# Kotomiya07/kuzushiji-vision

Measured on AMD Instinct MI355X. Metric: line-images/sec (train), higher is better.
Workload: dtype bf16; 1 GPU; TrOCR train step: ViT-B/16 (12L/768/12h/3072) on 64x640 crops (S_e=161) + RoBERTa decoder 6L/256/4h/768, V=4300 one-char vocab, labels [B,128], dropout 0.1, clip 1.0, RAdamScheduleFree; BASELINE.json configs[1]; per_gpu_batch=256, global_batch=256, parallelism=dp1

## Files before the change

include/kzv.h:

```cpp
#ifndef KZV_H
#define KZV_H
#include <stddef.h>
#include <stdint.h>

#ifdef __cplusplus
extern "C" {
#endif

#define KZV_OK 0
#define KZV_E_ARG (-1)
#define KZV_E_HIP (-2)
#define KZV_E_STATE (-3)

const char* kzv_last_error(void);
int kzv_version(void);

typedef struct kzv_config {
    int32_t image_h, image_w, patch_h, patch_w, channels;
    int32_t enc_hidden, enc_layers, enc_heads, enc_ffn;
    int32_t dec_hidden, dec_layers, dec_heads, dec_ffn;
    int32_t vocab, max_pos, type_vocab, pad_id;
    float enc_hidden_dropout, enc_attn_dropout, dec_hidden_dropout, dec_attn_dropout;
    float ln_eps;
} kzv_config;
// ... 342 lines not shown
                   float* dz, float* dgamma, float* dbeta, void* dy_bf16, int relu, int train, float* d_scratch, void* stream);
int kzv_ocr_maxpool_fwd(const void* x_bf16, void* out_bf16, unsigned char* idx, int N, int H, int W, int C, void* stream);
int kzv_ocr_maxpool_bwd(const float* dout, const unsigned char* idx, float* dx, int N, int H, int W, int C, void* stream);
int kzv_ocr_avgpool_fwd(const void* x_bf16, float* feat_f32, void* feat_bf16, int N, int HW, int C, void* stream);
int kzv_ocr_avgpool_bwd(const float* dfeat, float* dx, int N, int HW, int C, void* stream);
int kzv_ocr_lstm_cell_fwd(const float* gates, const float* b_hh, float* h_f32, void* h_bf16, int64_t ldh, int B, int H, void* stream);
int kzv_ocr_lstm_cell_bwd(const float* gates, const float* b_hh, const float* dh, int64_t lddh, void* dgates_bf16, int B, int H, void* stream);
int kzv_ocr_log_softmax(const float* x, float* lp, int rows, int C, void* stream);
int kzv_ocr_ctc(const float* lp, const int64_t* targets, int64_t ld_targets, const int64_t* input_lengths, const int64_t* target_lengths, int T,
                int B, int C, int blank, int zero_infinity, int max_target_len, float* d_scratch, float* d_nll, const float* d_gscale,
                float* d_dlogits, void* stream);
int kzv_ocr_smooth_l1_boxes(const float* pred, int max_boxes, const float* gt, int gt_boxes, const int32_t* counts, int B, float* d_loss,
                            float* d_dpred, void* stream);
int kzv_ocr_adam(float* p, const float* g, float* m, float* v, int64_t n, float lr, float beta1, float beta2, float eps, int step, void* stream);
int kzv_ocr_adam_dev(float* p, const float* g, float* m, float* v, int64_t n, float lr, float beta1, float beta2, float eps, const float* d_bc,
                     void* stream);
int kzv_ocr_cast_bf16(const float* x, void* out_bf16, int64_t n, void* stream);
int kzv_ocr_cast_transpose(const float* x, void* out_bf16, int rows, int cols, void* stream);

int kzv_prof_enable(int on, int capacity);
int kzv_prof_select(unsigned kind_mask);
int kzv_prof_collect(int kind, double* total_ms, double* total_flops, int64_t* launches);
int kzv_prof_sample(int stride);
int64_t kzv_prof_seen(int kind);
uint32_t kzv_drop_key(uint64_t seed, uint32_t site);

#define KZV_SITE_ENC_EMB 1u
#define KZV_SITE_ENC_LAYER(i, k) (16u + 4u * (uint32_t)(i) + (uint32_t)(k))
#define KZV_SITE_DEC_EMB 1000u
#define KZV_SITE_DEC_LAYER(i, k) (1016u + 8u * (uint32_t)(i) + (uint32_t)(k))

int kzv_debug_dropout_mask(uint32_t key, float p, int64_t rows, int64_t cols, int64_t ld_index, float* d_out, void* stream);
int kzv_debug_attn_dropout_mask(uint32_t key, float p, int64_t pairs, int32_t Sq, int32_t Sk, float* d_out, void* stream);

int kzv_set_cu_reserve(int n);
int kzv_get_cu_reserve(void);

int64_t kzv_scratch_growths(void);

typedef struct {
    int64_t src_off;
    int64_t tmp_off;
    int64_t hb_off, hk_off;
    int64_t vb_off, vk_off;
    int32_t in_h, in_w, new_h, new_w, paste_x, paste_y, hk_size, vk_size;
} kzv_line_desc;
int kzv_lanczos_coeffs(int in_size, int out_size, int32_t* bounds, int32_t* kk, int* ksize);
int kzv_preprocess_lines(const uint8_t* rgb, const kzv_line_desc* desc, const int32_t* coef, int n, int target_h, int target_w,
                         int64_t max_tmp_pixels, const float* lut256, uint8_t* tmp, float* out, void* stream);

typedef struct {
    float m[6];
    float blur[7];
    float contrast, brightness, noise_sigma;
    uint32_t noise_key;
    int32_t morph;
} kzv_augment_params;
int kzv_augment_lines(const float* in, const kzv_augment_params* params, int n, int H, int W, float* out, void* stream);

#ifdef __cplusplus
}
#endif
#endif
```

kuzushiji-vision_amd/csrc/gemm.hip:

```cpp
#include "kzv_common.h"
#include "../../include/kzv.h"
#include "kzv_host.h"
#include "gemm_nt.h"
#include "gemm_tn.h"

namespace {

constexpr int BK = 64;
constexpr int STAGE_BYTES = (128 + 128) * BK * 2;
constexpr int NT_LDS = 2 * STAGE_BYTES;

template <int N> __device__ __forceinline__ void wait_vmcnt() {
    if constexpr (N == 0) asm volatile("s_waitcnt vmcnt(0)" ::: "memory");
    else if constexpr (N == 4) asm volatile("s_waitcnt vmcnt(4)" ::: "memory");
    else if constexpr (N == 6) asm volatile("s_waitcnt vmcnt(6)" ::: "memory");
    else if constexpr (N == 8) asm volatile("s_waitcnt vmcnt(8)" ::: "memory");
    else if constexpr (N == 12) asm volatile("s_waitcnt vmcnt(12)" ::: "memory");
    else if constexpr (N == 16) asm volatile("s_waitcnt vmcnt(16)" ::: "memory");
    else static_assert(N == 0, "add the vmcnt literal");
}

template <int EPI, int WM, int WN, int NSTAGE, int KB, bool ASM_DMA>
__global__ __launch_bounds__(WM * WN * 64) void gemm_nt_kernel(const NtParams p) {
    constexpr int BM = WM * 64, BN = WN * 64, NW = WM * WN;
// ... 270 lines not shown
#pragma unroll
    for (int j = 0; j < 4; ++j)
#pragma unroll
        for (int i = 0; i < 4; ++i)
#pragma unroll
            for (int r = 0; r < 4; ++r) {
                const int n = wn * 64 + j * 16 + 4 * g + r, k = wk * 64 + i * 16 + l15;
                tile[n * 128 + ((((k >> 2) ^ (n & 31)) << 2) | (k & 3))] = acc[i][j][r];
            }
    __syncthreads();
    const bool interior = tnb * 128 + 128 <= p.n_store && tkb * 128 + 128 <= p.K;
    for (int it0 = 0; it0 < 64; it0 += 8) {
        float v[8];
#pragma unroll
        for (int u = 0; u < 8; ++u) {
            const int it = it0 + u;
            const int n = w * 32 + (it >> 1), k = (it & 1) * 64 + lane;
            v[u] = tile[n * 128 + ((((k >> 2) ^ (n & 31)) << 2) | (k & 3))];
        }
#pragma unroll
        for (int u = 0; u < 8; ++u) {
            const int it = it0 + u;
            const int n = w * 32 + (it >> 1), k = (it & 1) * 64 + lane;
            const int gn = tnb * 128 + n, gk = tkb * 128 + k;
            float* o = p.OUT + (int64_t)gn * p.ldo + gk;
            if (interior && p.splits > 1) atomicAdd(o, v[u]);
            else if (gn < p.n_store && gk < p.K) { if (p.splits == 1) *o += v[u]; else atomicAdd(o, v[u]); }
        }
    }
}

__global__ __launch_bounds__(256, 2) void gemm_tn_kernel(const TnParams p) { gemm_tn_body(p, blockIdx.x); }

constexpr int TN_GROUP_MAX = 40;
struct TnGroup { TnParams p[TN_GROUP_MAX]; int start[TN_GROUP_MAX + 1]; int n; };
__global__ __launch_bounds__(256, 2) void gemm_tn_group_kernel(const TnGroup g) {
    int i = 0;
#pragma unroll 1
    while (i + 1 < g.n && (int)blockIdx.x >= g.start[i + 1]) ++i;
    gemm_tn_body(g.p[i], (int)blockIdx.x - g.start[i]);
}

}

static int g_nt_schedule = -1;
static int g_nt_half_mask = -1;
static int nt_schedule() {
    if (g_nt_schedule < 0) {
        g_nt_schedule = kzv_env_int("KZV_NT_FREE", 0) != 0;
        if (kzv_env_int("KZV_NT_HALF", 0)) g_nt_schedule |= 2;
    }
    return g_nt_schedule;
}
static int nt_half_mask() {
    if (g_nt_half_mask < 0) g_nt_half_mask = kzv_env_int("KZV_NT_HALF_EPIS", 0x3f);
    return g_nt_half_mask;
}
extern "C" int kzv_set_nt_schedule(int n) { g_nt_schedule = n < 0 ? -1 : (n & 3); return KZV_OK; }
extern "C" int kzv_set_nt_half_epilogues(int mask) { g_nt_half_mask = mask; return KZV_OK; }

int kzv_nt_params(const kzv_gemm_nt_args* a, int epilogue, NtParams* out) {
    if (!a || !a->A || !a->B || !a->C) return kzv_fail(KZV_E_ARG, "gemm_nt: null operand");
    if (a->M <= 0 || a->N <= 0 || a->K <= 0) return kzv_fail(KZV_E_ARG, "gemm_nt: empty shape");
    if (a->K % 64) return kzv_fail(KZV_E_ARG, "gemm_nt: K must be a multiple of 64");
    if (a->N % 4 || a->ldc % 4) return kzv_fail(KZV_E_ARG, "gemm_nt: N and ldc must be multiples of 4");
    if (a->lda % 8 || a->ldb % 8) return kzv_fail(KZV_E_ARG, "gemm_nt: lda/ldb must be multiples of 8 (16-byte rows)");
    if (((uintptr_t)a->A | (uintptr_t)a->B | (uintptr_t)a->C) & 15) return kzv_fail(KZV_E_ARG, "gemm_nt: operands must be 16-byte aligned");
// ... 176 lines not shown
```

kuzushiji-vision_amd/csrc/gemm_tn.h:

```cpp
#pragma once
#include "kzv_common.h"

struct TnParams {
    const bf16_t* P; const bf16_t* Q; float* OUT; const void* zero16;
    int64_t ldp, ldq, ldo;
    int Mtok, N, K, n_store, splits, chunk;
    float* dbias;
};

inline bool tn_dma_offsets_fit(const TnParams& p) {
    return (uint64_t)64 * (uint64_t)p.ldp * 2 + (uint64_t)p.N * 2 <= 0xffffffffull && (uint64_t)64 * (uint64_t)p.ldq * 2 + (uint64_t)p.K * 2 <= 0xffffffffull;
}

int kzv_tn256_launch(const TnParams& p, hipStream_t s);

struct KzvTnFoldScope { explicit KzvTnFoldScope(hipStream_t stream); ~KzvTnFoldScope(); hipStream_t s; };

struct kzv_gemm_nt_args; struct kzv_gemm_tn_args;
int kzv_gemm_pair_launch(const kzv_gemm_nt_args* na, int epilogue, const kzv_gemm_tn_args* ta, hipStream_t s);
```

kuzushiji-vision_amd/csrc/gemm_tn256.hip:

```cpp
#include "kzv_common.h"
#include "../../include/kzv.h"
#include "kzv_host.h"
#include "gemm_tn.h"
#include "gemm_nt.h"
#include "gemm256_common.h"
#include "gemm_nt256p_body.h"
#include <vector>
#include <type_traits>

namespace {

constexpr int HT_BYTES = 64 * 256;
constexpr int BUF_BYTES = 4 * HT_BYTES;
constexpr int LDS_BYTES = 2 * BUF_BYTES;
constexpr int KP0 = 0, KP1 = 1, KQ0 = 2, KQ1 = 3;
#ifndef KZV_TN_F32_PARTIALS
constexpr size_t PART_FLOATS = 32768;
#else
constexpr size_t PART_FLOATS = 65536;
#endif

__global__ __launch_bounds__(512) void gemm_tn256_kernel(const TnParams p, float* part_ws) {
    extern __shared__ __attribute__((aligned(16))) char smem[];
    const int tid = threadIdx.x, lane = tid & 63;
    const int w = __builtin_amdgcn_readfirstlane(tid >> 6);
    const int g = lane >> 4, l15 = lane & 15;
    const int wr = w >> 2, wc = w & 3;
    const int tilesN = (p.N + 255) / 256, tilesK = (p.K + 255) / 256;
    const int per = tilesN * tilesK;
    const int id = xcd_remap(blockIdx.x, per * p.splits);
    const int split = id / per, rem = id - split * per;
    const int tnb = rem / tilesK, tkb = rem - tnb * tilesK;
    const int t_begin = split * p.chunk;
    const int t_end = min(p.Mtok, t_begin + p.chunk);
    const int nt = (t_end - t_begin) >> 6;

    const char* baseP = (const char*)(p.P + (int64_t)t_begin * p.ldp);
    const char* baseQ = (const char*)(p.Q + (int64_t)t_begin * p.ldq);
    const int64_t stepP = 64 * p.ldp * 2, stepQ = 64 * p.ldq * 2;
// ... 139 lines not shown
    }

    float* tile = (float*)smem;
    float* part = part_ws + (size_t)id * PART_FLOATS;
#pragma unroll
    for (int c = 0; c < 2; ++c) {
        __syncthreads();
#pragma unroll
        for (int j = 0; j < 4; ++j)
#pragma unroll
            for (int i = 0; i < 4; ++i)
#pragma unroll
                for (int r = 0; r < 4; ++r) {
                    const int ln = wr * 64 + j * 16 + 4 * g + r;
                    const int k = (i >> 1) * 128 + wc * 32 + (i & 1) * 16 + l15;
                    tile[ln * 256 + ((((k >> 2) ^ (ln & 31)) << 2) | (k & 3))] = acc[i][c * 4 + j][r];
                }
        __syncthreads();
#pragma unroll
        for (int it = 0; it < 16; ++it) {
            const int ln = w * 16 + it;
            const f32x4 v = *(const f32x4*)(tile + ln * 256 + ((lane ^ (ln & 31)) << 2));
            const int row = c * 128 + ln;
#ifndef KZV_TN_F32_PARTIALS
            typedef __attribute__((ext_vector_type(2))) unsigned u32x2p;
            __builtin_nontemporal_store((u32x2p){pack_bf2(v[0], v[1]), pack_bf2(v[2], v[3])}, (u32x2p*)((bf16_t*)part + row * 256 + lane * 4));
#else
            __builtin_nontemporal_store(v, (f32x4*)(part + row * 256 + lane * 4));
#endif
        }
    }
}

__device__ __forceinline__ void tn256f_body(const TnParams& p, float* const part, const int tnb, const int tkb, const int t_begin, const int nt,
                                            char* const smem) {
    const int tid = threadIdx.x, lane = tid & 63;
    const int w = __builtin_amdgcn_readfirstlane(tid >> 6);
    const int g = lane >> 4, l15 = lane & 15;
    const int wr = w >> 2, wc = w & 3;
    const int tilesK = (p.K + 255) / 256;

    const unsigned ldp2 = (unsigned)p.ldp * 2u, ldq2 = (unsigned)p.ldq * 2u;
    const char* baseP = (const char*)(p.P + (int64_t)t_begin * p.ldp);
    const char* baseQ = (const char*)(p.Q + (int64_t)t_begin * p.ldq);
    const int64_t stepP = 64 * (int64_t)ldp2, stepQ = 64 * (int64_t)ldq2;
    unsigned cP[2], cQ[2];
    {
        const int r = w * 4 + (lane >> 4);
        const int col2 = ((lane & 15) ^ ((r & 7) << 1)) * 16;
#pragma unroll
        for (int h = 0; h < 2; ++h) {
            cP[h] = (unsigned)r * ldp2 + (unsigned)min((tnb * 256 + h * 128) * 2 + col2, (p.N - 8) * 2);
            cQ[h] = (unsigned)r * ldq2 + (unsigned)min((tkb * 256 + h * 128) * 2 + col2, (p.K - 8) * 2);
        }
    }
    const unsigned ldsw = __builtin_amdgcn_readfirstlane((unsigned)(__SIZE_TYPE__)((KZV_LDS char*)smem) + (unsigned)w * 1024u);
    auto stP = [&](int buf, int h, int kt, int j) {
        const int kc = min(kt, nt - 1);
        glds16_s(cP[h], baseP + (int64_t)kc * stepP + (int64_t)j * 32 * ldp2, ldsw + (unsigned)((buf * 2 + h) * HT_BYTES + j * 8192));
    };
    auto stQ = [&](int buf, int h, int kt, int j) {
        const int kc = min(kt, nt - 1);
        glds16_s(cQ[h], baseQ + (int64_t)kc * stepQ + (int64_t)j * 32 * ldq2, ldsw + (unsigned)(65536 + (buf * 2 + h) * HT_BYTES + j * 8192));
    };

    f32x4 acc[4][8];
#pragma unroll
    for (int i = 0; i < 4; ++i)
// ... 85 lines not shown
        mm2(1, 1, 3, 0, Qs); KZV_TSB(); stP(BUF, 1, t + 2, 0); KZV_TSB();
        mm2(1, 1, 3, 1, Qs); KZV_TSB(); stP(BUF, 1, t + 2, 1); KZV_TSB();
#pragma unroll
        for (int j = 0; j < 4; ++j) {
            mm4(1, 0, j, Qf);
            KZV_TSB();
            if (!last) { rdP(BUF ^ 1, 0, j); if (j < 2) rdQ(BUF ^ 1, 0, j, Qs); }
            KZV_TSB();
        }
    };
    using I0 = std::integral_constant<int, 0>; using I1 = std::integral_constant<int, 1>;

#pragma unroll
    for (int b = 0; b < 2; ++b) {
        stP(b, 0, b, 0); stP(b, 0, b, 1); stQ(b, 0, b, 0); stQ(b, 0, b, 1);
        stQ(b, 1, b, 0); stQ(b, 1, b, 1); stP(b, 1, b, 0); stP(b, 1, b, 1);
    }
    vmcnt<12>();
    __builtin_amdgcn_s_barrier();
#pragma unroll
    for (int j = 0; j < 4; ++j) rdP(0, 0, j);
    rdQ(0, 0, 0, fqX); rdQ(0, 0, 1, fqX);
    for (int t = 0; t < nt; t += 2) {
        ktile(I0{}, fqX, fqY, t, t + 1 >= nt);
        if (t + 1 < nt) ktile(I1{}, fqY, fqX, t + 1, t + 2 >= nt);
    }
    vmcnt<0>();
#undef KZV_TSB

    if (bias_wave) {
#pragma unroll
        for (int j = 0; j < 8; ++j) {
            float v = bsum[j];
            v += __shfl_xor(v, 16, 64);
            v += __shfl_xor(v, 32, 64);
            const int n = tnb * 256 + (j >> 2) * 128 + wr * 64 + (j & 3) * 16 + l15;
            if (g == 0 && n < p.n_store) atomicAdd(p.dbias + n, v);
        }
    }

    float* tile = (float*)smem;
#pragma unroll
    for (int c = 0; c < 2; ++c) {
        __syncthreads();
#pragma unroll
        for (int j = 0; j < 4; ++j)
#pragma unroll
            for (int i = 0; i < 4; ++i)
#pragma unroll
                for (int r = 0; r < 4; ++r) {
                    const int ln = wr * 64 + j * 16 + 4 * g + r;
                    const int k = (i >> 1) * 128 + wc * 32 + (i & 1) * 16 + l15;
                    tile[ln * 256 + ((((k >> 2) ^ (ln & 31)) << 2) | (k & 3))] = acc[i][c * 4 + j][r];
                }
        __syncthreads();
#pragma unroll
        for (int it = 0; it < 16; ++it) {
            const int ln = w * 16 + it;
            const f32x4 v = *(const f32x4*)(tile + ln * 256 + ((lane ^ (ln & 31)) << 2));
            const int row = c * 128 + ln;
#ifndef KZV_TN_F32_PARTIALS
            typedef __attribute__((ext_vector_type(2))) unsigned u32x2p;
            __builtin_nontemporal_store((u32x2p){pack_bf2(v[0], v[1]), pack_bf2(v[2], v[3])}, (u32x2p*)((bf16_t*)part + row * 256 + lane * 4));
#else
            __builtin_nontemporal_store(v, (f32x4*)(part + row * 256 + lane * 4));
#endif
        }
    }
}

__global__ __launch_bounds__(512) void gemm_tn256f_kernel(const TnParams p, float* part_ws) {
    extern __shared__ __attribute__((aligned(16))) char smem[];
    const int tilesN = (p.N + 255) / 256, tilesK = (p.K + 255) / 256;
    const int per = tilesN * tilesK;
    const int id = xcd_remap(blockIdx.x, per * p.splits);
    const int split = id / per, rem = id - split * per;
    const int t_begin = split * p.chunk;
    const int t_end = min(p.Mtok, t_begin + p.chunk);
    tn256f_body(p, part_ws + (size_t)id * PART_FLOATS, rem / tilesK, rem % tilesK, t_begin, (t_end - t_begin) >> 6, smem);
}

struct PairPlan { unsigned short tile[256], split[256], t0[256], cnt[256]; };

template <int EPI>
__global__ __launch_bounds__(512) void gemm_pair_kernel(const NtParams pn, const int tiles, const int tilesN, const int strip_in, const TnParams pt,
                                                        float* part_ws, const int per, const PairPlan plan) {
    extern __shared__ __attribute__((aligned(16))) char smem[];
    nt256p_body<EPI, false>(pn, tiles, tilesN, strip_in, (int)blockIdx.x, (int)gridDim.x, smem);
    const int cnt = plan.cnt[blockIdx.x];
    if (cnt == 0) return;
    __syncthreads();
    const int tile = plan.tile[blockIdx.x], split = plan.split[blockIdx.x];
    const int tilesK = (pt.K + 255) / 256;
    tn256f_body(pt, part_ws + ((size_t)split * per + tile) * PART_FLOATS, tile / tilesK, tile % tilesK, (int)plan.t0[blockIdx.x] * 64, cnt, smem);
}

__global__ __launch_bounds__(256) void gemm_tn256_fold_kernel(const float* part_ws, float* OUT, int64_t ldo, int n_store, int K,
                                                             int tilesK, int per, int splits) {
    const int tile = blockIdx.x >> 6;
    const int row = (blockIdx.x & 63) * 4 + (threadIdx.x >> 6), k4 = (threadIdx.x & 63) * 4;
    const int tnb = tile / tilesK, tkb = tile - tnb * tilesK;
    const int gn = tnb * 256 + row, gk = tkb * 256 + k4;
    if (gn >= n_store || gk >= K) return;
    f32x4 s = (f32x4){0.f, 0.f, 0.f, 0.f};
#ifndef KZV_TN_F32_PARTIALS
    typedef __attribute__((ext_vector_type(2))) unsigned u32x2p;
#pragma unroll 4
    for (int sp = 0; sp < splits; ++sp) {
        const u32x2p u = __builtin_nontemporal_load((const u32x2p*)((const bf16_t*)(part_ws + ((size_t)sp * per + tile) * PART_FLOATS) + row * 256 + k4));
        s[0] += bf2f((bf16_t)(u[0] & 0xffffu)); s[1] += bf2f((bf16_t)(u[0] >> 16)); s[2] += bf2f((bf16_t)(u[1] & 0xffffu)); s[3] += bf2f((bf16_t)(u[1] >> 16));
    }
#else
// ... 75 lines not shown
    const int tok_tiles = p0.Mtok / 64;
    if (tiles < tn256_min_tiles() || p0.Mtok % 64 || tok_tiles < 2 || p0.N < 8 || p0.K < 8) return 0;
    if (!tn_dma_offsets_fit(p0)) return 0;
    TnParams p = p0;
    int cus = kzv_device_cus() - kzv_cu_reserve();
    { const int g = kzv_env_int("KZV_TN_CUS", 0); if (g > 0 && g < cus) cus = g; }
    int splits = cus / tiles;
    if (splits > tok_tiles / 8) splits = tok_tiles / 8;
    if (splits < 1) splits = 1;
    int chunk_tiles = (tok_tiles + splits - 1) / splits;
    if (chunk_tiles < 2) chunk_tiles = 2;
    splits = (tok_tiles + chunk_tiles - 1) / chunk_tiles;
    if (tok_tiles - (splits - 1) * chunk_tiles < 2) return 0;
    p.splits = splits; p.chunk = chunk_tiles * 64;
    if (p.K % 4 || p.ldo % 4 || ((uintptr_t)p.OUT & 15)) return 0;
    const size_t need = (size_t)tiles * splits * PART_FLOATS;
    const bool deferred = g_tn_defer > 0;
    bool same_out = false;
    for (const TnFold& e : g_tn_pending) same_out |= e.OUT == p.OUT;
    if (deferred && ((int)g_tn_pending.size() == TN_REGIONS - 1 || need > g_tn_region || same_out)) {
        if (tn_flush(s) != KZV_OK) return 0;
    }
    float* ws = tn_partials(need, deferred ? 1 + (int)g_tn_pending.size() : 0);
    if (!ws) return 0;
    if (tn_schedule()) kzv_launch_lds<gemm_tn256f_kernel>(dim3(tiles * splits), dim3(512), LDS_BYTES, s, p, ws);
    else kzv_launch_lds<gemm_tn256_kernel>(dim3(tiles * splits), dim3(512), LDS_BYTES, s, p, ws);
    if (deferred) {
        g_tn_pending.push_back(TnFold{ws, p.OUT, p.ldo, p.n_store, p.K, (p.K + 255) / 256, tiles, splits, 0});
        return 1;
    }
    hipLaunchKernelGGL(gemm_tn256_fold_kernel, dim3(tiles * 64), dim3(256), 0, s, ws, p.OUT, p.ldo, p.n_store, p.K,
                       (p.K + 255) / 256, tiles, splits);
    return 1;
}

int kzv_nt_params(const kzv_gemm_nt_args* a, int epilogue, NtParams* out);

namespace {
int g_pair = -1;
int pair_enabled() {
    if (g_pair < 0) g_pair = kzv_env_int("KZV_PAIR", 0) != 0;
    return g_pair;
}
double pair_ratio(int nk, int epilogue) {
    static int ov = -2;
    if (ov == -2) ov = kzv_env_int("KZV_PAIR_R", -1);
    const double drain = (epilogue == KZV_EPI_DGELU || epilogue == KZV_EPI_RESID) ? 5.0 : 2.5;
    const double r = 0.6 * (nk * 1.45 + drain) / 1.55;
    return ov >= 0 ? r * ov * 0.01 / 0.6 : r;
}
}

int kzv_gemm_pair_launch(const kzv_gemm_nt_args* na, int epilogue, const kzv_gemm_tn_args* ta, hipStream_t s) {
    if (!pair_enabled() || kzv_cu_reserve() != 0 || !tn_schedule() || kzv_device_cus() != 256) return 0;
    if (epilogue != KZV_EPI_BF16 && epilogue != KZV_EPI_F32 && epilogue != KZV_EPI_DGELU && epilogue != KZV_EPI_RESID) return 0;
    NtParams pn;
    if (kzv_nt_params(na, epilogue, &pn) != KZV_OK) return 0;
    const int tilesN = (pn.N + 255) / 256, tiles = ((pn.M + 255) / 256) * tilesN;
    if (pn.K < 128 || pn.K % 128 || tiles < 256) return 0;
    if (!nt_dma_offsets_fit(pn, 2)) return 0;
    TnParams pt{};
    pt.P = (const bf16_t*)ta->P; pt.Q = (const bf16_t*)ta->Q; pt.OUT = ta->OUT; pt.zero16 = kzv_zero_page();
    pt.ldp = ta->ldp; pt.ldq = ta->ldq; pt.ldo = ta->ldo; pt.Mtok = ta->Mtok; pt.N = ta->N; pt.K = ta->K;
    pt.n_store = ta->n_store > 0 ? ta->n_store : ta->N; pt.dbias = ta->dbias;
    if (!pt.P || !pt.Q || !pt.OUT || !pt.zero16) return 0;
    const int tilesKw = (pt.K + 255) / 256, tilesNw = (pt.N + 255) / 256, per = tilesNw * tilesKw;
// ... 80 lines not shown
```

kuzushiji-vision_amd/csrc/model_train.cpp:

```cpp
#include "model_internal.h"

static int g_dec_chain = -1;
int dec_chain_mode() {
    if (g_dec_chain < 0) { g_dec_chain = kzv_env_int("KZV_DEC_CHAIN", 2); if (g_dec_chain < 0 || g_dec_chain > 2) g_dec_chain = 2; }
    return g_dec_chain;
}
extern "C" int kzv_set_dec_chain(int on) {
    if (on < -1 || on > 2) return kzv_fail(KZV_E_ARG, "set_dec_chain: -1 (environment default), 0, 1 or 2");
    g_dec_chain = on;
    return KZV_OK;
}
static int g_head_ce = -1;
bool head_ce_mode() {
    if (g_head_ce < 0) g_head_ce = kzv_env_int("KZV_HEAD_CE", 1) != 0;
    return g_head_ce != 0;
}
extern "C" int kzv_set_head_ce(int on) {
    if (on < -1 || on > 1) return kzv_fail(KZV_E_ARG, "set_head_ce: -1 (environment default), 0 or 1");
    g_head_ce = on;
    return KZV_OK;
}
extern "C" int kzv_set_label_smoothing(kzv_model* m, float eps) {
    if (!m) return kzv_fail(KZV_E_ARG, "set_label_smoothing: null model");
    if (!(eps >= 0.f && eps < 1.f)) return kzv_fail(KZV_E_ARG, "set_label_smoothing: %g is not in [0, 1)", (double)eps);
    m->label_smoothing = eps;
    return KZV_OK;
}
extern "C" float kzv_get_label_smoothing(const kzv_model* m) { return m ? m->label_smoothing : 0.f; }

namespace {

struct WgradOpts {
    bool bias = true;
    int n = 0;
};
kzv_gemm_tn_args wgrad_args(const kzv_model* m, const Lin& l, const bf16_t* dY, int64_t ldy, const bf16_t* X, int64_t ldx, int Mtok, const WgradOpts& o) {
    kzv_gemm_tn_args a;
    memset(&a, 0, sizeof(a));
    a.P = dY; a.ldp = ldy; a.Q = X; a.ldq = ldx; a.OUT = m->G + l.w; a.ldo = l.K; a.Mtok = Mtok; a.N = o.n ? o.n : l.N; a.K = l.K; a.n_store = l.N;
    a.dbias = o.bias ? m->G + l.b : nullptr;
    return a;
}

int wgrad_flush(kzv_model* m, hipStream_t s) {
    if (m->wbatch.empty()) return KZV_OK;
    int rc = KZV_OK;
    for (size_t i = 0; i < m->wbatch.size() && rc == KZV_OK; i += 36)
        rc = kzv_gemm_tn_group(m->wbatch.data() + i, (int)std::min<size_t>(36, m->wbatch.size() - i), s);
    m->wbatch.clear();
    return rc;
}

enum { CLS_DY = 0, CLS_DBIG = 1, CLS_DQKV = 2, CLS_MISC = 3 };

int lin_wgrad(kzv_model* m, const Lin& l, int cls, hipStream_t s, const bf16_t* dY, int64_t ldy, const bf16_t* X, int64_t ldx, int Mtok,
              const WgradOpts& o = {}) {
    const kzv_gemm_tn_args a = wgrad_args(m, l, dY, ldy, X, ldx, Mtok, o);
    if (!m->use_side || (m->side_mode == 2 && !m->side_ok)) return kzv_gemm_tn(&a, s);
    if (hipEventRecord(m->ev_fork, s) != hipSuccess || hipStreamWaitEvent(m->side, m->ev_fork, 0) != hipSuccess)
        return kzv_fail(KZV_E_HIP, "wgrad_async: fork");
    const int rc = kzv_gemm_tn(&a, m->side);
    if (rc != KZV_OK) return rc;
    if (hipEventRecord(m->ev_done[cls], m->side) != hipSuccess) return kzv_fail(KZV_E_HIP, "wgrad_async: record");
    m->pending[cls] = true;
    return KZV_OK;
}
int lin_wgrad_batch(kzv_model* m, const Lin& l, int cls, hipStream_t s, const bf16_t* dY, int64_t ldy, const bf16_t* X, int64_t ldx, int Mtok,
                    const WgradOpts& o = {}) {
    if (m->use_side) return lin_wgrad(m, l, cls, s, dY, ldy, X, ldx, Mtok, o);
    m->wbatch.push_back(wgrad_args(m, l, dY, ldy, X, ldx, Mtok, o));
    return KZV_OK;
}
int wait_cls(kzv_model* m, int cls, hipStream_t s) {
    if (m->pending[cls]) {
        if (hipStreamWaitEvent(s, m->ev_done[cls], 0) != hipSuccess) return kzv_fail(KZV_E_HIP, "wait_cls");
        m->pending[cls] = false;
    }
    return KZV_OK;
}
int join_side(kzv_model* m, hipStream_t s) {
    for (int c = 0; c < 4; ++c) KZV_TRY(wait_cls(m, c, s));
// ... 474 lines not shown
```

kuzushiji-vision_amd/kzv/_lib.py:

```python
from __future__ import annotations

import ctypes as C
import os

_HERE = os.path.dirname(os.path.abspath(__file__))
LIB_PATH = os.environ.get("KZV_LIB") or os.path.join(_HERE, "libkzv.so")


class KzvError(RuntimeError):
    pass


class kzv_config(C.Structure):
    _fields_ = [(n, C.c_int32) for n in (
        "image_h", "image_w", "patch_h", "patch_w", "channels",
        "enc_hidden", "enc_layers", "enc_heads", "enc_ffn",
        "dec_hidden", "dec_layers", "dec_heads", "dec_ffn",
        "vocab", "max_pos", "type_vocab", "pad_id")] + [(n, C.c_float) for n in (
        "enc_hidden_dropout", "enc_attn_dropout", "dec_hidden_dropout", "dec_attn_dropout", "ln_eps")]


class kzv_opt_step(C.Structure):
    _fields_ = [("lr_t", C.c_float), ("ckp1", C.c_float), ("beta1", C.c_float), ("beta2", C.c_float),
                ("eps", C.c_float), ("weight_decay", C.c_float), ("bias_correction2", C.c_float),
# ... 173 lines not shown
    "kzv_gemm_tn": (C.c_int, [C.POINTER(kzv_gemm_tn_args), _P]),
    "kzv_layernorm_fwd": (C.c_int, [_P, _P, _P, _P, _P, _P, C.c_int, C.c_int, C.c_float, _P]),
    "kzv_layernorm_bwd": (C.c_int, [_P, C.c_int, _P, _P, _P, _P, C.c_int, _P, _P, C.c_int, C.c_int, _P]),
    "kzv_ln_fwd_ex": (C.c_int, [C.POINTER(kzv_ln_fwd_args), _P]),
    "kzv_ln_bwd_ex": (C.c_int, [C.POINTER(kzv_ln_bwd_args), _P]),
    "kzv_im2row": (C.c_int, [_P, _P] + [C.c_int] * 6 + [_P]),
    "kzv_embed_assemble": (C.c_int, [_P, _P, _P, _P, C.c_int, C.c_int, C.c_int, C.c_float, C.c_uint32, C.c_int, C.c_int, _P]),
    "kzv_embed_assemble_bwd": (C.c_int, [_P, _P, _P, _P, _P, C.c_int, C.c_int, C.c_int, C.c_float, C.c_uint32, C.c_int, C.c_int, _P]),
    "kzv_cast_drop_colsum": (C.c_int, [_P, _P, _P, C.c_int, C.c_int, C.c_float, C.c_uint32, _P, _P]),
    "kzv_colsum_bf16": (C.c_int, [_P, C.c_int64, _P, C.c_int, C.c_int, _P]),
    "kzv_dec_prepare": (C.c_int, [_P] + [C.c_int] * 5 + [_P, _P, _P, _P]),
    "kzv_embed_gather": (C.c_int, [_P, C.c_int, _P, _P, _P, _P, _P, C.c_int, C.c_int, C.c_int, _P]),
    "kzv_embed_scatter_bwd": (C.c_int, [_P, _P, C.c_int, _P, _P, _P, _P, C.c_int, C.c_int, C.c_int, C.c_int, _P]),
    "kzv_ce_fwd_bwd": (C.c_int, [_P, C.c_int64, _P] + [C.c_int] * 5 + [_P, _P, _P, _P]),
    "kzv_ce_fwd_bwd_ls": (C.c_int, [_P, C.c_int64, _P] + [C.c_int] * 5 + [_P, _P, _P, C.c_float, _P]),
    "kzv_copy_logits": (C.c_int, [_P, C.c_int64, _P, C.c_int, C.c_int, _P]),
    "kzv_cast_weights": (C.c_int, [C.POINTER(kzv_cast_desc), C.c_int, _P]),
    "kzv_attn_fwd": (C.c_int, [C.POINTER(kzv_attn_args), _P]),
    "kzv_attn_bwd": (C.c_int, [C.POINTER(kzv_attn_args), _P]),
    "kzv_attn_impl": (C.c_int, [C.POINTER(kzv_attn_args), C.c_int]),
    "kzv_attn_stream_fwd": (C.c_int, [C.POINTER(kzv_attn_args), _P]),
    "kzv_attn_stream_bwd": (C.c_int, [C.POINTER(kzv_attn_args), _P]),
    "kzv_attn_impl_ex": (C.c_int, [C.POINTER(kzv_attn_args), C.c_int, C.c_uint]),
    "kzv_attn_probs": (C.c_int, [C.POINTER(kzv_attn_probs_args), _P]),
    "kzv_token_scores": (C.c_int, [_P, C.c_int64, _P, C.c_int64, C.c_int, C.c_int, C.c_int, C.c_int, _P, _P, _P, _P]),
    "kzv_cross_attention": (C.c_int, [_P, C.c_int, _P, C.c_int64, _P, _P, _P]),
    "kzv_score_tokens": (C.c_int, [_P, _P, _P, _P, _P]),
    "kzv_score_tokens_topk": (C.c_int, [_P, C.c_int, _P, _P, _P]),
    "kzv_token_topk": (C.c_int, [_P, C.c_int64, C.c_int64, C.c_int, C.c_int, _P, _P, _P]),
    "kzv_edit_distance": (C.c_int, [C.POINTER(kzv_edit_args), _P]),
    "kzv_drop_key": (C.c_uint32, [C.c_uint64, C.c_uint32]),
    "kzv_debug_dropout_mask": (C.c_int, [C.c_uint32, C.c_float, C.c_int64, C.c_int64, C.c_int64, _P, _P]),
    "kzv_debug_attn_dropout_mask": (C.c_int, [C.c_uint32, C.c_float, C.c_int64, C.c_int32, C.c_int32, _P, _P]),
    "kzv_gemm_dgrad_wgrad": (C.c_int, [C.POINTER(kzv_gemm_nt_args), C.c_int, C.POINTER(kzv_gemm_tn_args), _P]),
    "kzv_set_pair": (C.c_int, [C.c_int]),
    "kzv_gemm_nt_f32": (C.c_int, [C.POINTER(kzv_gemm_nt_args), C.c_int, _P]),
    "kzv_gemm_tn_f32": (C.c_int, [C.POINTER(kzv_gemm_tn_args), _P]),
    "kzv_ocr_set_precision": (C.c_int, [C.c_int]),
    "kzv_ocr_nchw_to_nhwc": (C.c_int, [_P, _P, C.c_int, C.c_int, C.c_int, C.c_int, _P]),
    "kzv_ocr_im2col": (C.c_int, [_P, _P] + [C.c_int] * 9 + [_P]),
    "kzv_ocr_col2im": (C.c_int, [_P, _P] + [C.c_int] * 10 + [_P]),
    "kzv_ocr_conv_weight": (C.c_int, [_P, _P, _P] + [C.c_int] * 5 + [_P]),
    "kzv_ocr_conv_wgrad_unpack": (C.c_int, [_P, _P] + [C.c_int] * 5 + [_P]),
    "kzv_ocr_conv_weight_multi": (C.c_int, [C.c_int, _P, _P, _P, _P, _P]),
    "kzv_ocr_conv_wgrad_unpack_multi": (C.c_int, [C.c_int, _P, _P, _P, _P]),
    "kzv_ocr_bn_fwd": (C.c_int, [_P, C.c_int64, C.c_int, _P, _P, _P, _P, _P, _P, _P, _P, C.c_int, C.c_int, C.c_float, C.c_float, _P, _P]),
    "kzv_ocr_bn_bwd": (C.c_int, [_P, _P, _P, C.c_int64, C.c_int, _P, _P, _P, _P, _P, _P, _P, C.c_int, C.c_int, _P, _P]),
    "kzv_ocr_bn_scratch_floats": (C.c_int64, [C.c_int64, C.c_int]),
    "kzv_ocr_maxpool_fwd": (C.c_int, [_P, _P, _P, C.c_int, C.c_int, C.c_int, C.c_int, _P]),
    "kzv_ocr_maxpool_bwd": (C.c_int, [_P, _P, _P, C.c_int, C.c_int, C.c_int, C.c_int, _P]),
    "kzv_ocr_avgpool_fwd": (C.c_int, [_P, _P, _P, C.c_int, C.c_int, C.c_int, _P]),
    "kzv_ocr_avgpool_bwd": (C.c_int, [_P, _P, C.c_int, C.c_int, C.c_int, _P]),
    "kzv_ocr_lstm_cell_fwd": (C.c_int, [_P, _P, _P, _P, C.c_int64, C.c_int, C.c_int, _P]),
    "kzv_ocr_lstm_cell_bwd": (C.c_int, [_P, _P, _P, C.c_int64, _P, C.c_int, C.c_int, _P]),
    "kzv_ocr_log_softmax": (C.c_int, [_P, _P, C.c_int, C.c_int, _P]),
    "kzv_ocr_ctc": (C.c_int, [_P, _P, C.c_int64, _P, _P, C.c_int, C.c_int, C.c_int, C.c_int, C.c_int, C.c_int, _P, _P, _P, _P, _P]),
    "kzv_ocr_smooth_l1_boxes": (C.c_int, [_P, C.c_int, _P, C.c_int, _P, C.c_int, _P, _P, _P]),
    "kzv_ocr_adam": (C.c_int, [_P, _P, _P, _P, C.c_int64, C.c_float, C.c_float, C.c_float, C.c_float, C.c_int, _P]),
    "kzv_ocr_adam_dev": (C.c_int, [_P, _P, _P, _P, C.c_int64, C.c_float, C.c_float, C.c_float, C.c_float, _P, _P]),
    "kzv_ocr_cast_bf16": (C.c_int, [_P, _P, C.c_int64, _P]),
    "kzv_ocr_cast_transpose": (C.c_int, [_P, _P, C.c_int, C.c_int, _P]),
    "kzv_prof_enable": (C.c_int, [C.c_int, C.c_int]),
    "kzv_prof_select": (C.c_int, [C.c_uint]),
    "kzv_prof_sample": (C.c_int, [C.c_int]),
    "kzv_prof_seen": (C.c_int64, [C.c_int]),
    "kzv_set_cu_reserve": (C.c_int, [C.c_int]),
# ... 102 lines not shown
```

Before: 8499 img/s.

## Group small weight-gradient GEMMs into a split-K 256-tile kernel with fold

Batched weight-gradient GEMMs with fewer than 24 output tiles are routed into a new grouped 256x256 TN kernel. Each problem is split along the token dimension to fill the available CUs, and partials (fp32) and bias partials go to a workspace. A separate fold kernel reduces them in double precision and also handles tail tokens. This targets poor CU utilisation from small wgrad GEMMs in the older 128-tile grouped kernel, at the cost of extra workspace traffic and a second launch.

```diff
diff --git a/include/kzv.h b/include/kzv.h
--- a/include/kzv.h
+++ b/include/kzv.h
@@ -398,6 +398,7 @@
 
 int kzv_debug_dropout_mask(uint32_t key, float p, int64_t rows, int64_t cols, int64_t ld_index, float* d_out, void* stream);
 int kzv_debug_attn_dropout_mask(uint32_t key, float p, int64_t pairs, int32_t Sq, int32_t Sk, float* d_out, void* stream);
+int kzv_debug_gemm_tn_group(const kzv_gemm_tn_args* a, int n, int grouped256, void* stream);
 
 int kzv_set_cu_reserve(int n);
 int kzv_get_cu_reserve(void);
diff --git a/kuzushiji-vision_amd/csrc/gemm.hip b/kuzushiji-vision_amd/csrc/gemm.hip
--- a/kuzushiji-vision_amd/csrc/gemm.hip
+++ b/kuzushiji-vision_amd/csrc/gemm.hip
@@ -326,7 +326,6 @@
 
 __global__ __launch_bounds__(256, 2) void gemm_tn_kernel(const TnParams p) { gemm_tn_body(p, blockIdx.x); }
 
-constexpr int TN_GROUP_MAX = 40;
 struct TnGroup { TnParams p[TN_GROUP_MAX]; int start[TN_GROUP_MAX + 1]; int n; };
 __global__ __launch_bounds__(256, 2) void gemm_tn_group_kernel(const TnGroup g) {
     int i = 0;
diff --git a/kuzushiji-vision_amd/csrc/gemm_tn.h b/kuzushiji-vision_amd/csrc/gemm_tn.h
--- a/kuzushiji-vision_amd/csrc/gemm_tn.h
+++ b/kuzushiji-vision_amd/csrc/gemm_tn.h
@@ -12,6 +12,11 @@
     return (uint64_t)64 * (uint64_t)p.ldp * 2 + (uint64_t)p.N * 2 <= 0xffffffffull && (uint64_t)64 * (uint64_t)p.ldq * 2 + (uint64_t)p.K * 2 <= 0xffffffffull;
 }
 
+constexpr int TN_GROUP_MAX = 40;
+
+struct kzv_gemm_tn_args;
+int kzv_wgrad_group(const kzv_gemm_tn_args* a, int n, hipStream_t s);
+
 int kzv_tn256_launch(const TnParams& p, hipStream_t s);
 
 struct KzvTnFoldScope { explicit KzvTnFoldScope(hipStream_t stream); ~KzvTnFoldScope(); hipStream_t s; };
diff --git a/kuzushiji-vision_amd/csrc/gemm_tn256.hip b/kuzushiji-vision_amd/csrc/gemm_tn256.hip
--- a/kuzushiji-vision_amd/csrc/gemm_tn256.hip
+++ b/kuzushiji-vision_amd/csrc/gemm_tn256.hip
@@ -5,6 +5,7 @@
 #include "gemm_nt.h"
 #include "gemm256_common.h"
 #include "gemm_nt256p_body.h"
+#include <algorithm>
 #include <vector>
 #include <type_traits>
 
@@ -210,8 +211,9 @@
     }
 }
 
+template <bool GROUP = false>
 __device__ __forceinline__ void tn256f_body(const TnParams& p, float* const part, const int tnb, const int tkb, const int t_begin, const int nt,
-                                            char* const smem) {
+                                            char* const smem, float* const bias_part = nullptr) {
     const int tid = threadIdx.x, lane = tid & 63;
     const int w = __builtin_amdgcn_readfirstlane(tid >> 6);
     const int g = lane >> 4, l15 = lane & 15;
@@ -363,9 +365,10 @@
 #pragma unroll
         for (int j = 0; j < 8; ++j) {
             float v = bsum[j];
+            const int ln = (j >> 2) * 128 + wr * 64 + (j & 3) * 16 + l15, n = tnb * 256 + ln;
+            if constexpr (GROUP) { bias_part[g * 256 + ln] = v; continue; }
             v += __shfl_xor(v, 16, 64);
             v += __shfl_xor(v, 32, 64);
-            const int n = tnb * 256 + (j >> 2) * 128 + wr * 64 + (j & 3) * 16 + l15;
             if (g == 0 && n < p.n_store) atomicAdd(p.dbias + n, v);
         }
     }
@@ -390,6 +393,7 @@
             const int ln = w * 16 + it;
             const f32x4 v = *(const f32x4*)(tile + ln * 256 + ((lane ^ (ln & 31)) << 2));
             const int row = c * 128 + ln;
+            if constexpr (GROUP) { __builtin_nontemporal_store(v, (f32x4*)(part + row * 256 + lane * 4)); continue; }
 #ifndef KZV_TN_F32_PARTIALS
             typedef __attribute__((ext_vector_type(2))) unsigned u32x2p;
             __builtin_nontemporal_store((u32x2p){pack_bf2(v[0], v[1]), pack_bf2(v[2], v[3])}, (u32x2p*)((bf16_t*)part + row * 256 + lane * 4));
@@ -409,6 +413,72 @@
     const int t_begin = split * p.chunk;
     const int t_end = min(p.Mtok, t_begin + p.chunk);
     tn256f_body(p, part_ws + (size_t)id * PART_FLOATS, rem / tilesK, rem % tilesK, t_begin, (t_end - t_begin) >> 6, smem);
+}
+
+struct Tn256Group { TnParams p[TN_GROUP_MAX]; int start[TN_GROUP_MAX + 1]; int fstart[TN_GROUP_MAX + 1]; int n; };
+constexpr size_t PARTG_FLOATS = 65536, BIASG_FLOATS = 1024;
+
+__global__ __launch_bounds__(512) void gemm_tn256g_kernel(const Tn256Group g, float* part_ws, float* bias_ws) {
+    extern __shared__ __attribute__((aligned(16))) char smem[];
+    const int id = xcd_remap(blockIdx.x, gridDim.x);
+    int i = 0;
+#pragma unroll 1
+    while (i + 1 < g.n && id >= g.start[i + 1]) ++i;
+    const TnParams& p = g.p[i];
+    const int local = id - g.start[i];
+    const int tilesK = (p.K + 255) / 256, per = ((p.n_store + 255) / 256) * tilesK;
+    const int split = local / per, rem = local - split * per;
+    const int t_begin = split * p.chunk;
+    const int t_end = min(p.Mtok & ~63, t_begin + p.chunk);
+    tn256f_body<true>(p, part_ws + (size_t)id * PARTG_FLOATS, rem / tilesK, rem % tilesK, t_begin, (t_end - t_begin) >> 6, smem,
+                      bias_ws + (size_t)id * BIASG_FLOATS);
+}
+
+__global__ __launch_bounds__(256) void gemm_tn256g_fold_kernel(const Tn256Group g, const float* part_ws, const float* bias_ws) {
+    int i = 0;
+#pragma unroll 1
+    while (i + 1 < g.n && (int)blockIdx.x >= g.fstart[i + 1]) ++i;
+    const TnParams& p = g.p[i];
+    const int bid = blockIdx.x - g.fstart[i];
+    const int tile = bid >> 6;
+    const int row = (bid & 63) * 4 + (threadIdx.x >> 6), k4 = (threadIdx.x & 63) * 4;
+    const int tilesK = (p.K + 255) / 256, per = ((p.n_store + 255) / 256) * tilesK;
+    const int tnb = tile / tilesK, tkb = tile - tnb * tilesK;
+    const int gn = tnb * 256 + row, gk = tkb * 256 + k4;
+    if (gn >= p.n_store) return;
+    const int t_full = p.Mtok & ~63;
+    if (gk < p.K) {
+        double s[4] = {0., 0., 0., 0.};
+        const float* src = part_ws + (((size_t)g.start[i] + tile) * 256 + row) * 256 + k4;
+#pragma unroll 4
+        for (int sp = 0; sp < p.splits; ++sp) {
+            const f32x4 v = __builtin_nontemporal_load((const f32x4*)(src + (size_t)sp * per * PARTG_FLOATS));
+#pragma unroll
+            for (int q = 0; q < 4; ++q) s[q] += (double)v[q];
+        }
+        for (int t = t_full; t < p.Mtok; ++t) {
+            typedef __attribute__((ext_vector_type(2))) unsigned u32x2p;
+            const double a = (double)bf2f(p.P[(int64_t)t * p.ldp + gn]);
+            const u32x2p u = *(const u32x2p*)(p.Q + (int64_t)t * p.ldq + gk);
+            s[0] += a * (double)bf2f((bf16_t)(u[0] & 0xffffu)); s[1] += a * (double)bf2f((bf16_t)(u[0] >> 16));
+            s[2] += a * (double)bf2f((bf16_t)(u[1] & 0xffffu)); s[3] += a * (double)bf2f((bf16_t)(u[1] >> 16));
+        }
+        f32x4* o = (f32x4*)(p.OUT + (int64_t)gn * p.ldo + gk);
+        f32x4 r = *o;
+#pragma unroll
+        for (int q = 0; q < 4; ++q) r[q] = (float)((double)r[q] + s[q]);
+        *o = r;
+    }
+    if (p.dbias != nullptr && tkb == 0 && k4 == 0) {
+        double b = 0.;
+        const float* src = bias_ws + ((size_t)g.start[i] + tnb * tilesK) * BIASG_FLOATS + row;
+        for (int sp = 0; sp < p.splits; ++sp)
+            for (int kb = 0; kb < tilesK; ++kb)
+#pragma unroll
+                for (int q = 0; q < 4; ++q) b += (double)src[((size_t)sp * per + kb) * BIASG_FLOATS + q * 256];
+        for (int t = t_full; t < p.Mtok; ++t) b += (double)bf2f(p.P[(int64_t)t * p.ldp + gn]);
+        p.dbias[gn] = (float)((double)p.dbias[gn] + b);
+    }
 }
 
 struct PairPlan { unsigned short tile[256], split[256], t0[256], cnt[256]; };
@@ -550,6 +620,96 @@
     hipLaunchKernelGGL(gemm_tn256_fold_kernel, dim3(tiles * 64), dim3(256), 0, s, ws, p.OUT, p.ldo, p.n_store, p.K,
                        (p.K + 255) / 256, tiles, splits);
     return 1;
+}
+
+int kzv_gemm_tn_group(const kzv_gemm_tn_args* a, int n, hipStream_t s);
+
+namespace {
+KzvScratch g_tng_parts, g_tng_bias;
+int wgrad_group256() {
+    static int v = -1;
+    if (v < 0) v = kzv_env_int("KZV_WGRAD_GROUP256", 1) != 0;
+    return v;
+}
+bool tn256g_eligible(const kzv_gemm_tn_args& a, TnParams& p) {
+    if (!a.P || !a.Q || !a.OUT || a.Mtok < 128 || a.N < 8 || a.K < 8) return false;
+    if (a.N % 8 || a.K % 8 || a.ldp % 8 || a.ldq % 8 || a.ldo % 4) return false;
+    if (((uintptr_t)a.P | (uintptr_t)a.Q | (uintptr_t)a.OUT) & 15) return false;
+    p = TnParams{};
+    p.P = (const bf16_t*)a.P; p.Q = (const bf16_t*)a.Q; p.OUT = a.OUT; p.zero16 = nullptr;
+    p.ldp = a.ldp; p.ldq = a.ldq; p.ldo = a.ldo; p.Mtok = a.Mtok; p.N = a.N; p.K = a.K;
+    p.n_store = a.n_store > 0 ? a.n_store : a.N; p.dbias = a.dbias;
+    if (p.n_store > p.N || p.ldp < p.N || p.ldq < p.K || p.ldo < p.K) return false;
+    if (((p.n_store + 255) / 256) * ((p.K + 255) / 256) >= 24) return false;
+    return tn_dma_offsets_fit(p);
+}
+int tn256g_tiles(const TnParams& p) { return ((p.n_store + 255) / 256) * ((p.K + 255) / 256); }
+
+int tn256g_launch(const TnParams* ps, int n, hipStream_t s) {
+    int cus = kzv_device_cus() - kzv_cu_reserve();
+    { const int c = kzv_env_int("KZV_TN_CUS", 0); if (c > 0 && c < cus) cus = c; }
+    if (cus < 1) cus = 1;
+    Tn256Group g;
+    g.n = n;
+    double total = 0, work = 0;
+    for (int i = 0; i < n; ++i) total += (double)(ps[i].Mtok / 64) * tn256g_tiles(ps[i]);
+    int blocks = 0, fblocks = 0;
+    for (int i = 0; i < n; ++i) {
+        TnParams p = ps[i];
+        const int tiles = tn256g_tiles(p), stages = p.Mtok / 64;
+        int splits = (int)((double)cus * stages * tiles / total) / tiles;
+        if (splits > stages / 2) splits = stages / 2;
+        if (splits < 1) splits = 1;
+        int chunk = (stages + splits - 1) / splits;
+        splits = (stages + chunk - 1) / chunk;
+        while (splits > 1 && stages - (splits - 1) * chunk < 2) {
+            --splits;
+            chunk = (stages + splits - 1) / splits;
+            splits = (stages + chunk - 1) / chunk;
+        }
+        p.splits = splits; p.chunk = chunk * 64;
+        g.p[i] = p;
+        g.start[i] = blocks; blocks += tiles * splits;
+        g.fstart[i] = fblocks; fblocks += tiles * 64;
+        work += 2.0 * p.Mtok * p.n_store * p.K;
+    }
+    g.start[n] = blocks; g.fstart[n] = fblocks;
+    float* parts = (float*)g_tng_parts.get((size_t)blocks * PARTG_FLOATS * sizeof(float));
+    float* bias = (float*)g_tng_bias.get((size_t)blocks * BIASG_FLOATS * sizeof(float));
+    if (!parts || !bias) return kzv_fail(KZV_E_HIP, "gemm_tn256g: workspace");
+    KzvProfScope prof(1, work, s);
+    kzv_launch_lds<gemm_tn256g_kernel>(dim3(blocks), dim3(512), LDS_BYTES, s, g, parts, bias);
+    hipLaunchKernelGGL(gemm_tn256g_fold_kernel, dim3(fblocks), dim3(256), 0, s, g, (const float*)parts, (const float*)bias);
+    return kzv_check_launch("gemm_tn256g");
+}
+}
+
+int kzv_wgrad_group(const kzv_gemm_tn_args* a, int n, hipStream_t s) {
+    if (n <= 0) return KZV_OK;
+    std::vector<TnParams> el;
+    std::vector<kzv_gemm_tn_args> rest;
+    if (!a) return kzv_fail(KZV_E_ARG, "wgrad_group: null");
+    for (int i = 0; i < n; ++i) {
+        TnParams p;
+        bool ok = wgrad_group256() && tn256g_eligible(a[i], p);
+        for (size_t j = 0; ok && j < el.size(); ++j) ok = el[j].OUT != p.OUT && (!p.dbias || el[j].dbias != p.dbias);
+        if (ok) el.push_back(p); else rest.push_back(a[i]);
+    }
+    const int cus = std::max(1, kzv_device_cus() - kzv_cu_reserve());
+    for (size_t i = 0; i < el.size();) {
+        size_t j = i;
+        int tiles = 0;
+        while (j < el.size() && j - i < (size_t)TN_GROUP_MAX && (j == i || tiles + tn256g_tiles(el[j]) <= cus)) tiles += tn256g_tiles(el[j++]);
+        KZV_TRY_RC(tn256g_launch(el.data() + i, (int)(j - i), s));
+        i = j;
+    }
+    for (size_t i = 0; i < rest.size(); i += 36)
+        KZV_TRY_RC(kzv_gemm_tn_group(rest.data() + i, (int)std::min<size_t>(36, rest.size() - i), s));
+    return KZV_OK;
+}
+extern "C" int kzv_debug_gemm_tn_group(const kzv_gemm_tn_args* a, int n, int grouped256, void* stream) {
+    if (!a || n < 0) return kzv_fail(KZV_E_ARG, "debug_gemm_tn_group: null");
+    return grouped256 ? kzv_wgrad_group(a, n, (hipStream_t)stream) : kzv_gemm_tn_group(a, n, (hipStream_t)stream);
 }
 
 int kzv_nt_params(const kzv_gemm_nt_args* a, int epilogue, NtParams* out);
diff --git a/kuzushiji-vision_amd/csrc/model_train.cpp b/kuzushiji-vision_amd/csrc/model_train.cpp
--- a/kuzushiji-vision_amd/csrc/model_train.cpp
+++ b/kuzushiji-vision_amd/csrc/model_train.cpp
@@ -44,9 +44,7 @@
 
 int wgrad_flush(kzv_model* m, hipStream_t s) {
     if (m->wbatch.empty()) return KZV_OK;
-    int rc = KZV_OK;
-    for (size_t i = 0; i < m->wbatch.size() && rc == KZV_OK; i += 36)
-        rc = kzv_gemm_tn_group(m->wbatch.data() + i, (int)std::min<size_t>(36, m->wbatch.size() - i), s);
+    const int rc = kzv_wgrad_group(m->wbatch.data(), (int)m->wbatch.size(), s);
     m->wbatch.clear();
     return rc;
 }
diff --git a/kuzushiji-vision_amd/kzv/_lib.py b/kuzushiji-vision_amd/kzv/_lib.py
--- a/kuzushiji-vision_amd/kzv/_lib.py
+++ b/kuzushiji-vision_amd/kzv/_lib.py
@@ -229,6 +229,7 @@
     "kzv_drop_key": (C.c_uint32, [C.c_uint64, C.c_uint32]),
     "kzv_debug_dropout_mask": (C.c_int, [C.c_uint32, C.c_float, C.c_int64, C.c_int64, C.c_int64, _P, _P]),
     "kzv_debug_attn_dropout_mask": (C.c_int, [C.c_uint32, C.c_float, C.c_int64, C.c_int32, C.c_int32, _P, _P]),
+    "kzv_debug_gemm_tn_group": (C.c_int, [C.POINTER(kzv_gemm_tn_args), C.c_int, C.c_int, _P]),
     "kzv_gemm_dgrad_wgrad": (C.c_int, [C.POINTER(kzv_gemm_nt_args), C.c_int, C.POINTER(kzv_gemm_tn_args), _P]),
     "kzv_set_pair": (C.c_int, [C.c_int]),
     "kzv_gemm_nt_f32": (C.c_int, [C.POINTER(kzv_gemm_nt_args), C.c_int, _P]),
```

After: 8521 img/s, median of 3. No clear change (+0.3%).
